# Pointcept/Pointcept

Measured on AMD Instinct MI355X. Metric: scenes/sec (fwd+bwd+optimizer) PTv3 ScanNet-semseg @ ~100k pts, higher is better.
Workload: dtype bf16; 1 GPU; PT-v3m1 base (46.2M params) + seg head + CE + Lovasz, fwd+bwd+AdamW, 8 scenes x 102400 voxels per GPU, patch 1024, 4 orders; global_batch=8, parallelism=dp1, params=46167572, amp=bf16 autocast, points_per_gpu=819200, loss=CrossEntropy(ignore_index=-1) + LovaszSoftmax

## Files before the change

pointcept_amd/csrc/lovasz.hip:

```cpp
#include "ptc_common.h"
#include "voxel_keys.h"
#include "loss_rows.h"

#define LV_THREADS 256
#define LV_MAX_C PTC_LOVASZ_DENSE_MAX_C
#define LV_ONE 0x3f800000u
#define LV_STEP_BLOCKS 4096

__device__ __forceinline__ int64_t lv_key(float e, bool fg) { return (int64_t)(((uint64_t)(LV_ONE - __float_as_uint(e)) << 1) | (fg ? 1u : 0u)); }
__device__ __forceinline__ float lv_key_error(int64_t key) { return __uint_as_float(LV_ONE - (uint32_t)((uint64_t)key >> 1)); }

template <typename T>
__global__ void __launch_bounds__(LV_THREADS)
lovasz_keys_kernel(const T* __restrict__ logits, int64_t row_stride, const int64_t* __restrict__ target, int64_t n, int c,
                   int64_t ignore_index, int64_t* __restrict__ keys, int32_t* __restrict__ class_count) {
  __shared__ int32_t cnt[LV_MAX_C];
  if (threadIdx.x < LV_MAX_C) cnt[threadIdx.x] = 0;
  __syncthreads();
  const int64_t i = (int64_t)blockIdx.x * LV_THREADS + threadIdx.x;
  if (i < n) {
    const T* row = logits + i * row_stride;
    const int64_t t = target[i];
    const bool valid = t != ignore_index && t >= 0 && t < c;
    float m = -INFINITY;
// ... 109 lines not shown
  __shared__ double red[LV_THREADS];
  double acc = 0.0;
  for (int64_t i = threadIdx.x; i < n_partial; i += LV_THREADS) acc += partial[i];
  red[threadIdx.x] = acc;
  __syncthreads();
  for (int s = LV_THREADS / 2; s >= 1; s >>= 1) {
    if ((int)threadIdx.x < s) red[threadIdx.x] += red[threadIdx.x + s];
    __syncthreads();
  }
  if (threadIdx.x == 0) {
    int np = 0;
    for (int j = 0; j < c; ++j) np += class_count[j] > 0 ? 1 : 0;
    loss[0] = np > 0 ? (float)(red[0] / (double)np) : 0.f;
  }
}

template <typename T>
__global__ void __launch_bounds__(LV_THREADS)
lovasz_dlogits_kernel(const T* __restrict__ logits, int64_t row_stride, const int64_t* __restrict__ target,
                      const float* __restrict__ gprob, int64_t n, int c, int64_t ignore_index, float* __restrict__ dlogits) {
  const int64_t i = (int64_t)blockIdx.x * LV_THREADS + threadIdx.x;
  if (i >= n) return;
  const T* row = logits + i * row_stride;
  float* drow = dlogits + i * (int64_t)c;
  const int64_t t = target[i];
  const bool valid = t != ignore_index && t >= 0 && t < c;
  if (!valid) {
    for (int j = 0; j < c; ++j) drow[j] = 0.f;
    return;
  }
  float m = -INFINITY;
  for (int j = 0; j < c; ++j) m = fmaxf(m, ptc_to_float(row[j]));
  float ssum = 0.f;
  for (int j = 0; j < c; ++j) ssum += __expf(ptc_to_float(row[j]) - m);
  const float inv = 1.f / ssum;
  float dot = 0.f;
  for (int j = 0; j < c; ++j) dot += gprob[(int64_t)j * n + i] * (__expf(ptc_to_float(row[j]) - m) * inv);
  for (int j = 0; j < c; ++j) {
    const float p = __expf(ptc_to_float(row[j]) - m) * inv;
    drow[j] = p * (gprob[(int64_t)j * n + i] - dot);
  }
}

template <typename T, int VB>
__global__ void __launch_bounds__(LV_THREADS)
lovasz_dlogits_rows_kernel(const T* __restrict__ logits, int64_t row_stride, const int64_t* __restrict__ target,
                           const float* __restrict__ gprob, int64_t n, int c, int64_t ignore_index, float* __restrict__ dlogits, int a16) {
  extern __shared__ __attribute__((aligned(16))) unsigned char smem[];
  const int64_t row0 = (int64_t)blockIdx.x * LV_THREADS, i = row0 + threadIdx.x;
  if (i < n) {
    float* drow = reinterpret_cast<float*>(smem) + (int)threadIdx.x * c;
    const int64_t t = target[i];
    const bool valid = t != ignore_index && t >= 0 && t < c;
    if (!valid) {
#pragma unroll
      for (int j = 0; j < LR_CP; ++j) if (j < c) drow[j] = 0.f;
    } else {
      float v[LR_CP], gp[LR_CP];
      lr_load_row<T, VB>(logits + i * row_stride, c, v);
#pragma unroll
      for (int j = 0; j < LR_CP; ++j) gp[j] = j < c ? gprob[(int64_t)j * n + i] : 0.f;
      float m = -INFINITY;
#pragma unroll
      for (int j = 0; j < LR_CP; ++j) if (j < c) m = fmaxf(m, v[j]);
      float ssum = 0.f;
#pragma unroll
      for (int j = 0; j < LR_CP; ++j) if (j < c) { v[j] = __expf(v[j] - m); ssum += v[j]; }
      const float inv = 1.f / ssum;
      float dot = 0.f;
#pragma unroll
      for (int j = 0; j < LR_CP; ++j) if (j < c) dot += gp[j] * (v[j] * inv);
#pragma unroll
      for (int j = 0; j < LR_CP; ++j) {
        if (j < c) {
          const float p = v[j] * inv;
          drow[j] = p * (gp[j] - dot);
        }
      }
    }
  }
  __syncthreads();
  const int64_t rows = (n - row0) < LV_THREADS ? (n - row0) : LV_THREADS;
  lr_copy_out<float>(smem, dlogits + row0 * c, (int)rows * c, a16 != 0);
}

struct LvLayout {
  size_t keys, order, fg, scan, gprob, partial, count, sort_ws, scan_ws, total;
  int64_t n_partial;
};
static LvLayout lv_layout(int64_t n, int c) {
  LvLayout L;
  const size_t nc = (size_t)(n > 0 ? n : 1) * (size_t)c;
  int64_t g = ptc_cdiv(n > 0 ? n : 1, LV_THREADS);
  if (g > LV_STEP_BLOCKS / c) g = LV_STEP_BLOCKS / c;
  L.n_partial = (g > 0 ? g : 1) * c;
  size_t o = 0;
  L.keys = o; o += ptc_align_up(nc * 8, 256);
  L.order = o; o += ptc_align_up(nc * 8, 256);
  L.fg = o; o += ptc_align_up(nc * 4, 256);
  L.scan = o; o += ptc_align_up(nc * 8, 256);
  L.gprob = o; o += ptc_align_up(nc * 4, 256);
  L.partial = o; o += ptc_align_up((size_t)L.n_partial * 8, 256);
  L.count = o; o += 256;
  L.sort_ws = o; o += ptc_align_up(ptc_sort_keys_workspace_bytes(n, c), 256);
  L.scan_ws = o; o += ptc_align_up(ptc_exclusive_scan_workspace_bytes((int64_t)nc), 256);
  L.total = o;
  return L;
}

extern "C" size_t ptc_lovasz_softmax_workspace_bytes(int64_t n, int c) {
  if (n < 0 || c < 1 || c > LV_MAX_C) return 0;
  return lv_layout(n, c).total;
}

extern "C" int ptc_lovasz_softmax(const void* logits, int64_t row_stride, const int64_t* target, int64_t n, int c, int dtype,
                                  int64_t ignore_index, float* loss, float* dlogits, void* workspace,
                                  size_t workspace_bytes, ptc_stream_t stream) {
  PTC_REQUIRE(n >= 0 && c >= 1 && row_stride >= c, PTC_EINVAL, "ptc_lovasz_softmax: bad sizes");
  PTC_REQUIRE(c <= LV_MAX_C, PTC_EUNSUPPORTED, "ptc_lovasz_softmax: c=%d > %d classes", c, LV_MAX_C);
  PTC_REQUIRE(n < (1ll << 31), PTC_EUNSUPPORTED, "ptc_lovasz_softmax: n >= 2^31");
  PTC_REQUIRE(loss != nullptr, PTC_EINVAL, "ptc_lovasz_softmax: null loss");
  hipStream_t s = (hipStream_t)stream;
  if (n == 0) {
    PTC_HIP(hipMemsetAsync(loss, 0, sizeof(float), s));
    return PTC_OK;
  }
  PTC_REQUIRE(logits && target && dlogits && workspace, PTC_EINVAL, "ptc_lovasz_softmax: null buffer");
  const LvLayout L = lv_layout(n, c);
  PTC_REQUIRE(workspace_bytes >= L.total, PTC_EWORKSPACE, "ptc_lovasz_softmax: workspace %zu < %zu", workspace_bytes, L.total);
  char* ws = (char*)workspace;
  int64_t* keys = (int64_t*)(ws + L.keys);
  int64_t* order = (int64_t*)(ws + L.order);
  int32_t* fg = (int32_t*)(ws + L.fg);
  int64_t* scan = (int64_t*)(ws + L.scan);
  float* gprob = (float*)(ws + L.gprob);
  double* partial = (double*)(ws + L.partial);
  int32_t* count = (int32_t*)(ws + L.count);
  const int64_t nc = n * (int64_t)c;
  const unsigned grid_n = (unsigned)ptc_cdiv(n, LV_THREADS), grid_nc = (unsigned)ptc_cdiv(nc, LV_THREADS);

  const bool rows = c <= LR_CP;
  const int vb = lr_vec_bytes(logits, row_stride, c, ptc_dtype_size(dtype));
  PTC_HIP(hipMemsetAsync(count, 0, 256, s));
  if (rows) {
    PTC_DISPATCH_DTYPE(dtype, T, LR_DISPATCH_VB(vb, VB, hipLaunchKernelGGL((lovasz_keys_rows_kernel<T, VB>), dim3(grid_n), dim3(LV_THREADS), 0, s,
                                                                         (const T*)logits, row_stride, target, n, c, ignore_index, keys, count)))
  } else {
    PTC_DISPATCH_DTYPE(dtype, T, hipLaunchKernelGGL(lovasz_keys_kernel<T>, dim3(grid_n), dim3(LV_THREADS), 0, s, (const T*)logits,
                                                     row_stride, target, n, c, ignore_index, keys, count))
  }
  PTC_CHECK_LAUNCH("lovasz_keys_kernel");
  int rc = ptc_sort_keys_ex(keys, n, c, 1, 31, order, nullptr, keys, ws + L.sort_ws, L.scan_ws - L.sort_ws, stream);
  if (rc != PTC_OK) return rc;
  hipLaunchKernelGGL(lovasz_fg_kernel, dim3(grid_nc), dim3(LV_THREADS), 0, s, keys, nc, fg);
  PTC_CHECK_LAUNCH("lovasz_fg_kernel");
  rc = ptc_exclusive_scan_i32(fg, nc, scan, ws + L.scan_ws, L.total - L.scan_ws, stream);
  if (rc != PTC_OK) return rc;
  hipLaunchKernelGGL(lovasz_step_kernel, dim3((unsigned)(L.n_partial / c), (unsigned)c), dim3(LV_THREADS), 0, s, keys, order, scan, count, n, c, gprob,
                     partial);
  PTC_CHECK_LAUNCH("lovasz_step_kernel");
  hipLaunchKernelGGL(lovasz_finish_kernel, dim3(1), dim3(LV_THREADS), 0, s, partial, L.n_partial, count, c, loss);
  PTC_CHECK_LAUNCH("lovasz_finish_kernel");
  if (rows) {
    const int a16 = ((uintptr_t)dlogits & 15) == 0;
    const size_t lds = (size_t)LV_THREADS * c * sizeof(float);
    PTC_DISPATCH_DTYPE(dtype, T, LR_DISPATCH_VB(vb, VB, hipLaunchKernelGGL((lovasz_dlogits_rows_kernel<T, VB>), dim3(grid_n), dim3(LV_THREADS), lds, s,
                                                                         (const T*)logits, row_stride, target, gprob, n, c, ignore_index, dlogits,
                                                                         a16)))
  } else {
    PTC_DISPATCH_DTYPE(dtype, T, hipLaunchKernelGGL(lovasz_dlogits_kernel<T>, dim3(grid_n), dim3(LV_THREADS), 0, s, (const T*)logits,
                                                     row_stride, target, gprob, n, c, ignore_index, dlogits))
  }
  PTC_CHECK_LAUNCH("lovasz_dlogits_kernel");
  return PTC_OK;
}

#define LW_MAX_C PTC_LOVASZ_MAX_C
#define LW_RV 16
#define LW_TILE_BYTES (32 * 1024)

__global__ void __launch_bounds__(LV_THREADS)
lovasz_count_kernel(const int64_t* __restrict__ target, int64_t n, int c, int64_t ignore_index, int32_t* __restrict__ class_count) {
  __shared__ int32_t cnt[LW_MAX_C];
  for (int j = threadIdx.x; j < c; j += LV_THREADS) cnt[j] = 0;
  __syncthreads();
  for (int64_t i = (int64_t)blockIdx.x * LV_THREADS + threadIdx.x; i < n; i += (int64_t)gridDim.x * LV_THREADS) {
    const int64_t t = target[i];
    if (t != ignore_index && t >= 0 && t < c) atomicAdd(&cnt[(int)t], 1);
  }
  __syncthreads();
  for (int j = threadIdx.x; j < c; j += LV_THREADS)
    if (cnt[j] != 0) atomicAdd(&class_count[j], cnt[j]);
}

__global__ void __launch_bounds__(LV_THREADS)
lovasz_rank_kernel(const int32_t* __restrict__ class_count, int c, int32_t* __restrict__ row_of, int32_t* __restrict__ class_of,
                   int32_t* __restrict__ n_present) {
  __shared__ int32_t wsum[LV_THREADS / 64];
  constexpr int PER = LW_MAX_C / LV_THREADS;
  const int lane = ptc_lane(), wave = threadIdx.x >> 6, j0 = (int)threadIdx.x * PER;
  bool f[PER];
  int32_t mine = 0;
#pragma unroll
  for (int q = 0; q < PER; ++q) {
    f[q] = j0 + q < c && class_count[j0 + q] > 0;
    mine += f[q] ? 1 : 0;
  }
  int32_t incl = mine;
#pragma unroll
  for (int o = 1; o < 64; o <<= 1) {
// ... 319 lines not shown
```

pointcept_amd/csrc/ptc_common.h:

```cpp
#pragma once
#include <hip/hip_runtime.h>
#include <stdint.h>
#include <stdio.h>
#include <stdarg.h>
#include "../../include/ptcore.h"

#define PTC_WAVE 64

void ptc_set_error(const char* fmt, ...);

#define PTC_REQUIRE(cond, code, ...)      \
  do {                                    \
    if (!(cond)) {                        \
      ptc_set_error(__VA_ARGS__);         \
      return (code);                      \
    }                                     \
  } while (0)

#define PTC_CHECK_LAUNCH(name)                                                        \
  do {                                                                                \
    hipError_t e__ = hipGetLastError();                                               \
    if (e__ != hipSuccess) {                                                          \
      ptc_set_error("%s: launch failed: %s", (name), hipGetErrorString(e__));         \
      return PTC_EHIP;                                                                \
// ... 54 lines not shown
#define PTC_DISPATCH_DTYPE(dtype, T, ...)                 \
  switch (dtype) {                                        \
    case PTC_F32: { using T = float; __VA_ARGS__; } break; \
    case PTC_F16: { using T = f16_t; __VA_ARGS__; } break; \
    case PTC_BF16: { using T = bf16_t; __VA_ARGS__; } break; \
    default: ptc_set_error("bad dtype %d", (int)(dtype)); return PTC_EINVAL; \
  }

static inline size_t ptc_dtype_size(int dtype) { return dtype == PTC_F32 ? 4 : 2; }

#define PTC_SWZ64(s) (((((s) >> 1) & 1) << 2) | (((s) >> 2) & 3))

__device__ __forceinline__ int ptc_lane() { return threadIdx.x & 63; }

__device__ __forceinline__ uint32_t ptc_float_enc(float f) {
  const uint32_t b = __float_as_uint(f);
  return (b & 0x80000000u) ? ~b : (b | 0x80000000u);
}
__device__ __forceinline__ float ptc_float_dec(uint32_t k) { return __uint_as_float((k & 0x80000000u) ? (k & 0x7fffffffu) : ~k); }

__device__ __forceinline__ float ptc_dist2(float ax, float ay, float az, float bx, float by, float bz) {
#pragma clang fp contract(off)
  const float dx = ax - bx, dy = ay - by, dz = az - bz;
  const float xx = dx * dx, yy = dy * dy, zz = dz * dz;
  return (xx + yy) + zz;
}

template <int I> struct ptc_int { static constexpr int value = I; };
template <int N, int I = 0, typename F> __device__ __forceinline__ void ptc_static_for(F&& f) {
  if constexpr (I < N) {
    f(ptc_int<I>{});
    ptc_static_for<N, I + 1>(f);
  }
}

__host__ __device__ __forceinline__ void ptc_rope_pair(float u, float v, float cs, float sn, float& ru, float& rv) {
  ru = fmaf(u, cs, -(v * sn));
  rv = fmaf(v, cs, u * sn);
}

#ifndef PTC_FAST_GELU
#define PTC_FAST_GELU 1
#endif
__device__ __forceinline__ float ptc_gelu_cdf(float z) {
#if PTC_FAST_GELU
  const float t = fminf(fabsf(z) * 0.70710678118654752f, 3.95f);
  float r = -4.535858889e-05f;
  r = fmaf(r, t, 4.455075312e-04f);
  r = fmaf(r, t, -1.489441160e-03f);
  r = fmaf(r, t, -7.746305554e-04f);
  r = fmaf(r, t, 2.825368195e-02f);
  r = fmaf(r, t, -1.484816155e-01f);
  r = fmaf(r, t, -9.184163932e-01f);
  r = fmaf(r, t, -1.627908593e+00f);
  const float h = __builtin_amdgcn_exp2f(fmaf(r, t, -1.0f));
  return z < 0.f ? h : 1.0f - h;
#else
  return 0.5f * (1.f + erff(z * 0.70710678118654752f));
#endif
}
__device__ __forceinline__ float ptc_gelu(float z) {
#if PTC_FAST_GELU
  return z * ptc_gelu_cdf(z);
#else
  return 0.5f * z * (1.f + erff(z * 0.70710678118654752f));
#endif
}
__device__ __forceinline__ float ptc_gelu_grad(float z) {
#if PTC_FAST_GELU
  return fmaf(z * 0.3989422804014327f, __builtin_amdgcn_exp2f(z * z * -0.72134752044448170f), ptc_gelu_cdf(z));
#else
  return 0.5f * (1.f + erff(z * 0.70710678118654752f)) + z * 0.3989422804014327f * __expf(-0.5f * z * z);
#endif
}

#ifdef __HIPCC__
#define PTC_WAVES_PER_EU(lo, hi) __attribute__((amdgpu_waves_per_eu(lo, hi)))
#else
#define PTC_WAVES_PER_EU(lo, hi)
#endif

int ptc_sort_keys_ex(const int64_t* keys, int64_t n, int k, int begin_bit, int end_bit, int64_t* order, int64_t* inverse,
                     int64_t* sorted_keys, void* workspace, size_t workspace_bytes, ptc_stream_t stream);
struct PtcCellGrid;
int ptc_cell_grid_params(const float* xyz, int64_t n, double radius, uint32_t* mm, PtcCellGrid* grid, ptc_stream_t stream);
int ptc_cell_grid_sort(const float* xyz, const int64_t* keys, int64_t n, int end_bit, int64_t* order, int64_t* sorted_keys, float4* sxyz,
                       void* scratch, size_t scratch_bytes, ptc_stream_t stream);
```

pointcept_amd/csrc/scan_sort.hip:

```cpp
#include "ptc_common.h"

__device__ __forceinline__ int64_t wave_inclusive_scan_i64(int64_t v) {
  const int lane = ptc_lane();
#pragma unroll
  for (int d = 1; d < 64; d <<= 1) {
    int lo = __shfl_up((int)(uint32_t)(v & 0xffffffffll), d, 64);
    int hi = __shfl_up((int)(uint32_t)((uint64_t)v >> 32), d, 64);
    int64_t o = (int64_t)(((uint64_t)(uint32_t)hi << 32) | (uint32_t)lo);
    if (lane >= d) v += o;
  }
  return v;
}

#define SCAN_THREADS 256
#define SCAN_ITEMS 8
#define SCAN_TILE (SCAN_THREADS * SCAN_ITEMS)

__device__ __forceinline__ int64_t block_exclusive_scan_i64(int64_t v, int64_t* total, int64_t* smem ) {
  const int lane = ptc_lane(), wave = threadIdx.x >> 6;
  int64_t inc = wave_inclusive_scan_i64(v);
  if (lane == 63) smem[wave] = inc;
  __syncthreads();
  if (threadIdx.x == 0) {
    int64_t run = 0;
    for (int w = 0; w < SCAN_THREADS / 64; ++w) { int64_t t = smem[w]; smem[w] = run; run += t; }
    smem[4] = run;
  }
  __syncthreads();
  int64_t excl = inc - v + smem[wave];
  *total = smem[4];
  __syncthreads();
  return excl;
}

__global__ void __launch_bounds__(SCAN_THREADS)
scan_tile_sums_kernel(const int32_t* __restrict__ in, int64_t n, int64_t* __restrict__ tile_sums) {
  __shared__ int64_t smem[5];
  const int64_t base = (int64_t)blockIdx.x * SCAN_TILE + (int64_t)threadIdx.x * SCAN_ITEMS;
  int64_t s = 0;
#pragma unroll
  for (int j = 0; j < SCAN_ITEMS; ++j) { int64_t i = base + j; if (i < n) s += in[i]; }
  int64_t total;
  block_exclusive_scan_i64(s, &total, smem);
  if (threadIdx.x == 0) tile_sums[blockIdx.x] = total;
}

__global__ void __launch_bounds__(SCAN_THREADS)
scan_tile_sums_scan_kernel(int64_t* __restrict__ tile_sums, int64_t n_tiles) {
  __shared__ int64_t smem[5];
  int64_t carry = 0;
  for (int64_t c = 0; c < n_tiles; c += SCAN_THREADS) {
    int64_t i = c + threadIdx.x;
    int64_t v = (i < n_tiles) ? tile_sums[i] : 0;
    int64_t total;
    int64_t ex = block_exclusive_scan_i64(v, &total, smem);
    if (i < n_tiles) tile_sums[i] = carry + ex;
    carry += total;
  }
}

__global__ void __launch_bounds__(SCAN_THREADS)
scan_apply_kernel(const int32_t* __restrict__ in, int64_t n, const int64_t* __restrict__ tile_offsets,
                  int64_t* __restrict__ out) {
  __shared__ int64_t smem[5];
  const int64_t base = (int64_t)blockIdx.x * SCAN_TILE + (int64_t)threadIdx.x * SCAN_ITEMS;
  int32_t v[SCAN_ITEMS];
  int64_t s = 0;
#pragma unroll
  for (int j = 0; j < SCAN_ITEMS; ++j) { int64_t i = base + j; v[j] = (i < n) ? in[i] : 0; s += v[j]; }
  int64_t total;
  int64_t ex = block_exclusive_scan_i64(s, &total, smem) + tile_offsets[blockIdx.x];
#pragma unroll
  for (int j = 0; j < SCAN_ITEMS; ++j) { int64_t i = base + j; if (i < n) out[i] = ex; ex += v[j]; }
}

#define SCAN1_THREADS 1024
#define SCAN1_ITEMS 16
#define SCAN1_MAX (SCAN1_THREADS * SCAN1_ITEMS)
__global__ void __launch_bounds__(SCAN1_THREADS)
scan_single_kernel(const int32_t* __restrict__ in, int64_t n, int64_t* __restrict__ out) {
  __shared__ int64_t wsum[SCAN1_THREADS / 64], wex[SCAN1_THREADS / 64 + 1];
  const int lane = ptc_lane(), wave = threadIdx.x >> 6;
  int64_t carry = 0;
  for (int64_t sweep = 0; sweep < n; sweep += (int64_t)SCAN1_THREADS * SCAN1_ITEMS) {
    const int64_t base = sweep + (int64_t)threadIdx.x * SCAN1_ITEMS;
    int32_t v[SCAN1_ITEMS];
    int64_t s = 0;
#pragma unroll
    for (int j = 0; j < SCAN1_ITEMS; ++j) { const int64_t i = base + j; v[j] = (i < n) ? in[i] : 0; s += v[j]; }
    const int64_t inc = wave_inclusive_scan_i64(s);
    if (lane == 63) wsum[wave] = inc;
    __syncthreads();
    if (wave == 0) {
      const int64_t w = lane < SCAN1_THREADS / 64 ? wsum[lane] : 0;
      const int64_t winc = wave_inclusive_scan_i64(w);
      if (lane < SCAN1_THREADS / 64) wex[lane] = winc - w;
      if (lane == SCAN1_THREADS / 64 - 1) wex[SCAN1_THREADS / 64] = winc;
    }
    __syncthreads();
    int64_t ex = carry + wex[wave] + inc - s;
#pragma unroll
    for (int j = 0; j < SCAN1_ITEMS; ++j) { const int64_t i = base + j; if (i < n) out[i] = ex; ex += v[j]; }
    carry += wex[SCAN1_THREADS / 64];
    __syncthreads();
  }
}

static int64_t scan_num_tiles(int64_t n) { return ptc_cdiv(n > 0 ? n : 1, SCAN_TILE); }

extern "C" size_t ptc_exclusive_scan_workspace_bytes(int64_t n) {
  return ptc_align_up((size_t)scan_num_tiles(n) * sizeof(int64_t), 256);
}

static int exclusive_scan_i32(const int32_t* in, int64_t n, int64_t* out, void* ws, hipStream_t s) {
  if (n <= 0) return PTC_OK;
  if (n <= SCAN1_MAX) {
    hipLaunchKernelGGL(scan_single_kernel, dim3(1), dim3(SCAN1_THREADS), 0, s, in, n, out);
    PTC_CHECK_LAUNCH("scan_single_kernel");
    return PTC_OK;
  }
  int64_t tiles = scan_num_tiles(n);
  int64_t* tile_sums = (int64_t*)ws;
  hipLaunchKernelGGL(scan_tile_sums_kernel, dim3((unsigned)tiles), dim3(SCAN_THREADS), 0, s, in, n, tile_sums);
  PTC_CHECK_LAUNCH("scan_tile_sums_kernel");
  hipLaunchKernelGGL(scan_tile_sums_scan_kernel, dim3(1), dim3(SCAN_THREADS), 0, s, tile_sums, tiles);
  PTC_CHECK_LAUNCH("scan_tile_sums_scan_kernel");
  hipLaunchKernelGGL(scan_apply_kernel, dim3((unsigned)tiles), dim3(SCAN_THREADS), 0, s, in, n, tile_sums, out);
  PTC_CHECK_LAUNCH("scan_apply_kernel");
  return PTC_OK;
}

extern "C" int ptc_exclusive_scan_i32(const int32_t* in, int64_t n, int64_t* out, void* workspace,
                                      size_t workspace_bytes, ptc_stream_t stream) {
  PTC_REQUIRE(n >= 0, PTC_EINVAL, "ptc_exclusive_scan_i32: n < 0");
  if (n == 0) return PTC_OK;
  PTC_REQUIRE(in && out && workspace, PTC_EINVAL, "ptc_exclusive_scan_i32: null buffer");
  PTC_REQUIRE(workspace_bytes >= ptc_exclusive_scan_workspace_bytes(n), PTC_EWORKSPACE,
              "ptc_exclusive_scan_i32: workspace %zu < %zu", workspace_bytes, ptc_exclusive_scan_workspace_bytes(n));
  return exclusive_scan_i32(in, n, out, workspace, (hipStream_t)stream);
}

#define RS_THREADS 256
#define RS_WAVES (RS_THREADS / 64)
#define RS_ITERS 16
#define RS_TILE (RS_THREADS * RS_ITERS)
#define RS_RADIX 256
#ifndef RS_PACK
#define RS_PACK 1
#endif

__device__ __forceinline__ uint32_t rs_digit(uint64_t key, int shift, uint32_t mask) {
  return (uint32_t)(key >> shift) & mask;
}

__global__ void __launch_bounds__(RS_THREADS)
rs_histogram_kernel(const uint64_t* __restrict__ keys, int64_t n, int shift, uint32_t mask,
                    int n_blocks, int32_t* __restrict__ hist) {
  __shared__ int32_t lh[RS_RADIX];
  const int row = blockIdx.y, blk = blockIdx.x;
  lh[threadIdx.x] = 0;
  __syncthreads();
  const uint64_t* k = keys + (int64_t)row * n;
  const int64_t base = (int64_t)blk * RS_TILE;
#pragma unroll 4
  for (int it = 0; it < RS_ITERS; ++it) {
    int64_t i = base + (int64_t)it * RS_THREADS + threadIdx.x;
    if (i < n) atomicAdd(&lh[rs_digit(k[i], shift, mask)], 1);
  }
  __syncthreads();
  hist[((int64_t)row * RS_RADIX + threadIdx.x) * n_blocks + blk] = lh[threadIdx.x];
}

template <bool FIRST, bool PACK>
__global__ void __launch_bounds__(RS_THREADS)
rs_scatter_kernel(const uint64_t* __restrict__ keys_in, const uint32_t* __restrict__ idx_in, int64_t n,
                  int shift, uint32_t mask, int n_blocks, const int64_t* __restrict__ offsets,
                  uint64_t* __restrict__ keys_out, uint32_t* __restrict__ idx_out, int idx_bits, uint64_t key_mask) {
  __shared__ int32_t wave_hist[RS_WAVES][RS_RADIX];
  __shared__ int64_t glob[RS_RADIX];
  __shared__ uint64_t skeys[RS_TILE];
  __shared__ uint32_t svals[PACK ? 1 : RS_TILE];
  const int row = blockIdx.y, blk = blockIdx.x;
  const int lane = ptc_lane(), wave = threadIdx.x >> 6;
  for (int i = threadIdx.x; i < RS_WAVES * RS_RADIX; i += RS_THREADS) (&wave_hist[0][0])[i] = 0;
  glob[threadIdx.x] = offsets[((int64_t)row * RS_RADIX + threadIdx.x) * n_blocks + blk] - (int64_t)row * n;
  __syncthreads();

  const uint64_t* k = keys_in + (int64_t)row * n;
  const uint32_t* ix = (FIRST || PACK) ? nullptr : idx_in + (int64_t)row * n;
  const int dshift = shift + ((PACK && FIRST) ? idx_bits : 0);
  const int64_t base = (int64_t)blk * RS_TILE + (int64_t)wave * (RS_ITERS * 64);
  const uint64_t lt_mask = (lane == 0) ? 0ull : (~0ull >> (64 - lane));

  uint64_t key[RS_ITERS];
  uint32_t val[RS_ITERS];
  int32_t rank[RS_ITERS];
#pragma unroll
  for (int it = 0; it < RS_ITERS; ++it) {
    const int64_t i = base + (int64_t)it * 64 + lane;
    const bool valid = i < n;
    key[it] = valid ? k[i] : ~0ull;
    if (PACK && FIRST && valid) key[it] = ((key[it] & key_mask) << idx_bits) | (uint64_t)i;
    val[it] = (valid && !PACK) ? (FIRST ? (uint32_t)i : ix[i]) : 0u;
    const uint32_t d = rs_digit(key[it], dshift, mask);
    uint64_t peers = __ballot(valid);
#pragma unroll
    for (int b = 0; b < 8; ++b) {
      const bool bit = (d >> b) & 1u;
      const uint64_t bal = __ballot(bit);
      peers &= bit ? bal : ~bal;
    }
    int32_t before = 0;
    if (valid) {
      before = wave_hist[wave][d];
      rank[it] = before + __popcll(peers & lt_mask);
    } else {
      rank[it] = 0;
    }
    __builtin_amdgcn_wave_barrier();
    if (valid && (peers & lt_mask) == 0ull) wave_hist[wave][d] = before + __popcll(peers);
    __builtin_amdgcn_wave_barrier();
  }
  __syncthreads();
  int32_t run = 0;
#pragma unroll
  for (int w = 0; w < RS_WAVES; ++w) { int32_t c = wave_hist[w][threadIdx.x]; wave_hist[w][threadIdx.x] = run; run += c; }
  __shared__ int32_t lstart[RS_RADIX];
  __shared__ int32_t wsum[RS_WAVES];
  {
    int32_t incl = run;
#pragma unroll
    for (int o = 1; o < 64; o <<= 1) {
      const int32_t v = __shfl_up(incl, o, 64);
      if (lane >= o) incl += v;
    }
    if (lane == 63) wsum[wave] = incl;
    __syncthreads();
    int32_t base_w = 0;
#pragma unroll
    for (int w = 0; w < RS_WAVES; ++w) base_w += (w < wave) ? wsum[w] : 0;
    lstart[threadIdx.x] = base_w + incl - run;
  }
  __syncthreads();
#pragma unroll
  for (int it = 0; it < RS_ITERS; ++it) {
    const int64_t i = base + (int64_t)it * 64 + lane;
    if (i < n) {
      const uint32_t d = rs_digit(key[it], dshift, mask);
      const int lp = lstart[d] + wave_hist[wave][d] + rank[it];
      skeys[lp] = key[it];
      if (!PACK) svals[lp] = val[it];
    }
  }
  __syncthreads();
  uint64_t* ko = keys_out + (int64_t)row * n;
  uint32_t* io = PACK ? nullptr : idx_out + (int64_t)row * n;
  const int64_t tile0 = (int64_t)blk * RS_TILE;
  const int cnt = (int)((n - tile0) < RS_TILE ? (n - tile0) : RS_TILE);
  for (int j = threadIdx.x; j < cnt; j += RS_THREADS) {
    const uint64_t kk = skeys[j];
// ... 1 lines not shown
    const int64_t dst = glob[d] + (j - lstart[d]);
    ko[dst] = kk;
    if (!PACK) io[dst] = svals[j];
  }
}

__global__ void __launch_bounds__(256)
rs_finalize_kernel(const uint32_t* __restrict__ idx, const uint64_t* __restrict__ packed, uint64_t idx_mask, int idx_bits, int64_t n, int k,
                   int64_t* __restrict__ order, int64_t* __restrict__ inverse, const uint64_t* plain,
                   int64_t* sorted_keys) {
  const int64_t total = n * k;
  const int64_t stride = (int64_t)gridDim.x * blockDim.x;
  for (int64_t t = (int64_t)blockIdx.x * blockDim.x + threadIdx.x; t < total; t += stride) {
    const int64_t row = t / n, i = t - row * n;
    const uint64_t word = packed ? packed[t] : 0ull;
    const int64_t src = packed ? (int64_t)(word & idx_mask) : (idx ? (int64_t)idx[t] : i);
    order[t] = src;
    if (inverse) inverse[row * n + src] = i;
    if (sorted_keys) sorted_keys[t] = (int64_t)(packed ? (word >> idx_bits) : plain[t]);
  }
}

static int rs_num_blocks(int64_t n) { return (int)ptc_cdiv(n > 0 ? n : 1, RS_TILE); }

struct RsLayout {
  size_t keysA, keysB, idxA, idxB, hist, offs, scan, total;
};
static RsLayout rs_layout(int64_t n, int k) {
  RsLayout L;
  const size_t nk = (size_t)(n > 0 ? n : 1) * (size_t)k;
  const size_t nh = (size_t)k * RS_RADIX * (size_t)rs_num_blocks(n);
  size_t o = 0;
  L.keysA = o; o += ptc_align_up(nk * 8, 256);
  L.keysB = o; o += ptc_align_up(nk * 8, 256);
  L.idxA = o; o += ptc_align_up(nk * 4, 256);
  L.idxB = o; o += ptc_align_up(nk * 4, 256);
  L.hist = o; o += ptc_align_up(nh * 4, 256);
  L.offs = o; o += ptc_align_up(nh * 8, 256);
  L.scan = o; o += ptc_exclusive_scan_workspace_bytes((int64_t)nh);
  L.total = o;
  return L;
}

extern "C" size_t ptc_sort_keys_workspace_bytes(int64_t n, int k) { return rs_layout(n, k).total; }

extern "C" int ptc_sort_keys(const int64_t* keys, int64_t n, int k, int begin_bit, int end_bit,
                             int64_t* order, int64_t* inverse, void* workspace, size_t workspace_bytes,
                             ptc_stream_t stream) {
  return ptc_sort_keys_ex(keys, n, k, begin_bit, end_bit, order, inverse, nullptr, workspace, workspace_bytes, stream);
}

int ptc_sort_keys_ex(const int64_t* keys, int64_t n, int k, int begin_bit, int end_bit, int64_t* order, int64_t* inverse,
                     int64_t* sorted_keys, void* workspace, size_t workspace_bytes, ptc_stream_t stream) {
  PTC_REQUIRE(n >= 0 && k >= 1, PTC_EINVAL, "ptc_sort_keys: bad n=%lld k=%d", (long long)n, k);
  PTC_REQUIRE(begin_bit >= 0 && end_bit <= 64 && begin_bit <= end_bit, PTC_EINVAL,
              "ptc_sort_keys: bad bit range [%d,%d)", begin_bit, end_bit);
  PTC_REQUIRE(n < (1ll << 32), PTC_EUNSUPPORTED, "ptc_sort_keys: n >= 2^32");
  if (n == 0) return PTC_OK;
  PTC_REQUIRE(keys && order && workspace, PTC_EINVAL, "ptc_sort_keys: null buffer");
  const RsLayout L = rs_layout(n, k);
  PTC_REQUIRE(workspace_bytes >= L.total, PTC_EWORKSPACE, "ptc_sort_keys: workspace %zu < %zu", workspace_bytes, L.total);
  hipStream_t s = (hipStream_t)stream;
  char* ws = (char*)workspace;
  uint64_t* kbuf[2] = {(uint64_t*)(ws + L.keysA), (uint64_t*)(ws + L.keysB)};
  uint32_t* ibuf[2] = {(uint32_t*)(ws + L.idxA), (uint32_t*)(ws + L.idxB)};
  int32_t* hist = (int32_t*)(ws + L.hist);
  int64_t* offs = (int64_t*)(ws + L.offs);
  void* scan_ws = ws + L.scan;
  const int nb = rs_num_blocks(n);
  const int64_t nh = (int64_t)k * RS_RADIX * nb;

  const uint64_t* cur_k = (const uint64_t*)keys;
  const uint32_t* cur_i = nullptr;
  int out = 0;
  bool first = true;
  int idx_bits = 1;
  while (((int64_t)1 << idx_bits) < n) ++idx_bits;
  const bool pack = RS_PACK && (end_bit - begin_bit) > 0 && end_bit + idx_bits <= 64;
  const uint64_t key_mask = end_bit >= 64 ? ~0ull : (((uint64_t)1 << end_bit) - 1);
  for (int shift = begin_bit; shift < end_bit; shift += 8) {
    const int bits = (end_bit - shift) < 8 ? (end_bit - shift) : 8;
    const uint32_t mask = (1u << bits) - 1u;
    const int hshift = shift + ((pack && !first) ? idx_bits : 0);
    hipLaunchKernelGGL(rs_histogram_kernel, dim3(nb, k), dim3(RS_THREADS), 0, s, cur_k, n, hshift, mask, nb, hist);
    PTC_CHECK_LAUNCH("rs_histogram_kernel");
    int rc = exclusive_scan_i32(hist, nh, offs, scan_ws, s);
    if (rc != PTC_OK) return rc;
#define RS_SCATTER(F, P)                                                                                                                          \
    hipLaunchKernelGGL((rs_scatter_kernel<F, P>), dim3(nb, k), dim3(RS_THREADS), 0, s, cur_k, cur_i, n, (P && !F) ? shift + idx_bits : shift, mask, nb, \
                       offs, kbuf[out], ibuf[out], idx_bits, key_mask)
    if (pack) { if (first) RS_SCATTER(true, true); else RS_SCATTER(false, true); }
    else { if (first) RS_SCATTER(true, false); else RS_SCATTER(false, false); }
#undef RS_SCATTER
    PTC_CHECK_LAUNCH("rs_scatter_kernel");
    cur_k = kbuf[out];
    cur_i = ibuf[out];
    out ^= 1;
    first = false;
  }
  {
    const int64_t total = n * k;
    int64_t grid = ptc_cdiv(total, 256);
    if (grid > 4096) grid = 4096;
    const bool packed_out = pack && !first;
    hipLaunchKernelGGL(rs_finalize_kernel, dim3((unsigned)grid), dim3(256), 0, s, packed_out ? nullptr : cur_i, packed_out ? cur_k : nullptr,
                       (((uint64_t)1 << idx_bits) - 1), idx_bits, n, k, order, inverse, cur_k, sorted_keys);
    PTC_CHECK_LAUNCH("rs_finalize_kernel");
  }
  return PTC_OK;
}
```

Before: 229.7 scenes/s.

## Compact Lovasz sort to live entries and use single flat device-sized radix sort

Adds a flat Lovasz-softmax path. For each class it computes a cutoff, the minimum error among that class's foreground points. Only entries at or above that cutoff (plus foreground entries) are compacted into packed 64-bit words (class | error | fg | index), which are then sorted with a radix sort whose length comes from a device-side count. This replaces the full n*c per-class key sort, since entries below the cutoff contribute no Lovasz gradient, and it cuts the sort from many per-class rows to one packed pass over the live subset. The cost is extra passes over the logits (cut, live count, compaction), added small scans and launches, and correctness that depends on the cutoff argument and on the bit packing fitting in 64 bits.

```diff
diff --git a/pointcept_amd/csrc/lovasz.hip b/pointcept_amd/csrc/lovasz.hip
--- a/pointcept_amd/csrc/lovasz.hip
+++ b/pointcept_amd/csrc/lovasz.hip
@@ -215,6 +215,337 @@
   __syncthreads();
   const int64_t rows = (n - row0) < LV_THREADS ? (n - row0) : LV_THREADS;
   lr_copy_out<float>(smem, dlogits + row0 * c, (int)rows * c, a16 != 0);
+}
+
+struct LvState {
+  int32_t count[LV_MAX_C];
+  int32_t live[LV_MAX_C];
+  uint32_t cut[LV_MAX_C];
+  int64_t seg_start[LV_MAX_C];
+  int32_t fg_start[LV_MAX_C];
+  int64_t m;
+  int32_t n_present;
+};
+#define LF_ITEMS 8
+#define LF_TILE (LV_THREADS * LF_ITEMS)
+
+__device__ __forceinline__ void lv_row_errors(float (&v)[LR_CP], int c, int64_t t, bool valid) {
+  float m = -INFINITY;
+#pragma unroll
+  for (int j = 0; j < LR_CP; ++j) if (j < c) m = fmaxf(m, v[j]);
+  float ssum = 0.f;
+#pragma unroll
+  for (int j = 0; j < LR_CP; ++j) if (j < c) { v[j] = __expf(v[j] - m); ssum += v[j]; }
+  const float inv = 1.f / ssum;
+#pragma unroll
+  for (int j = 0; j < LR_CP; ++j) {
+    if (j < c) {
+      const float p = v[j] * inv;
+      const float e = valid ? (j == t ? 1.f - p : p) : 0.f;
+      v[j] = fminf(fmaxf(e, 0.f), 1.f);
+    }
+  }
+}
+
+__device__ __forceinline__ uint32_t lv_live_mask(const float (&e)[LR_CP], int c, int64_t t, bool valid, const uint32_t* cut) {
+  uint32_t mask = 0;
+#pragma unroll
+  for (int j = 0; j < LR_CP; ++j)
+    if (j < c && ((valid && j == t) || __float_as_uint(e[j]) >= cut[j])) mask |= 1u << j;
+  return mask;
+}
+
+template <typename T, int VB>
+__global__ void __launch_bounds__(LV_THREADS)
+lovasz_cut_kernel(const T* __restrict__ logits, int64_t row_stride, const int64_t* __restrict__ target, int64_t n, int c,
+                  int64_t ignore_index, LvState* __restrict__ st) {
+  __shared__ int32_t cnt[LR_CP];
+  __shared__ uint32_t cut[LR_CP];
+  if (threadIdx.x < LR_CP) { cnt[threadIdx.x] = 0; cut[threadIdx.x] = 0xffffffffu; }
+  __syncthreads();
+  const int64_t i = (int64_t)blockIdx.x * LV_THREADS + threadIdx.x;
+  if (i < n) {
+    const int64_t t = target[i];
+    if (t != ignore_index && t >= 0 && t < c) {
+      float v[LR_CP];
+      lr_load_row<T, VB>(logits + i * row_stride, c, v);
+      lv_row_errors(v, c, t, true);
+      atomicAdd(&cnt[(int)t], 1);
+      atomicMin(&cut[(int)t], __float_as_uint(lr_pick(v, (int)t)));
+    }
+  }
+  __syncthreads();
+  if (threadIdx.x < c && cnt[threadIdx.x] != 0) {
+    atomicAdd(&st->count[threadIdx.x], cnt[threadIdx.x]);
+    atomicMin(&st->cut[threadIdx.x], cut[threadIdx.x]);
+  }
+}
+
+template <typename T, int VB>
+__global__ void __launch_bounds__(LV_THREADS)
+lovasz_live_count_kernel(const T* __restrict__ logits, int64_t row_stride, const int64_t* __restrict__ target, int64_t n, int c,
+                         int64_t ignore_index, LvState* __restrict__ st, int32_t* __restrict__ block_live) {
+  __shared__ int32_t lc[LR_CP];
+  __shared__ uint32_t cut[LR_CP];
+  if (threadIdx.x < LR_CP) { lc[threadIdx.x] = 0; cut[threadIdx.x] = threadIdx.x < c ? st->cut[threadIdx.x] : 0xffffffffu; }
+  __syncthreads();
+  const int64_t i = (int64_t)blockIdx.x * LV_THREADS + threadIdx.x;
+  uint32_t mask = 0;
+  if (i < n) {
+    float v[LR_CP];
+    lr_load_row<T, VB>(logits + i * row_stride, c, v);
+    const int64_t t = target[i];
+    const bool valid = t != ignore_index && t >= 0 && t < c;
+    lv_row_errors(v, c, t, valid);
+    mask = lv_live_mask(v, c, t, valid, cut);
+  }
+  for (int j = 0; j < c; ++j) {
+    const uint64_t b = __ballot((mask >> j) & 1u);
+    if (ptc_lane() == 0 && b != 0ull) atomicAdd(&lc[j], __popcll(b));
+  }
+  __syncthreads();
+  if (threadIdx.x < c && lc[threadIdx.x] != 0) atomicAdd(&st->live[threadIdx.x], lc[threadIdx.x]);
+  if (threadIdx.x == 0) {
+    int32_t total = 0;
+    for (int j = 0; j < c; ++j) total += lc[j];
+    block_live[blockIdx.x] = total;
+  }
+}
+
+__global__ void lovasz_plan_kernel(LvState* __restrict__ st, int c) {
+  int64_t seg = 0;
+  int32_t fg = 0, np = 0;
+  for (int j = 0; j < c; ++j) {
+    st->seg_start[j] = seg;
+    st->fg_start[j] = fg;
+    seg += st->live[j];
+    fg += st->count[j];
+    np += st->count[j] > 0 ? 1 : 0;
+  }
+  st->m = seg;
+  st->n_present = np;
+}
+
+template <typename T, int VB>
+__global__ void __launch_bounds__(LV_THREADS)
+lovasz_compact_kernel(const T* __restrict__ logits, int64_t row_stride, const int64_t* __restrict__ target, int64_t n, int c,
+                      int64_t ignore_index, const LvState* __restrict__ st, const int64_t* __restrict__ block_off, int pbits,
+                      int64_t cap, uint64_t* __restrict__ words) {
+  __shared__ uint32_t cut[LR_CP];
+  __shared__ int32_t wsum[LV_THREADS / 64];
+  if (threadIdx.x < LR_CP) cut[threadIdx.x] = threadIdx.x < c ? st->cut[threadIdx.x] : 0xffffffffu;
+  __syncthreads();
+  const int64_t i = (int64_t)blockIdx.x * LV_THREADS + threadIdx.x;
+  const int lane = ptc_lane(), wave = threadIdx.x >> 6;
+  float v[LR_CP];
+  uint32_t mask = 0;
+  int64_t t = -1;
+  bool valid = false;
+  if (i < n) {
+    lr_load_row<T, VB>(logits + i * row_stride, c, v);
+    t = target[i];
+    valid = t != ignore_index && t >= 0 && t < c;
+    lv_row_errors(v, c, t, valid);
+    mask = lv_live_mask(v, c, t, valid, cut);
+  }
+  const int32_t mine = __popc(mask);
+  int32_t incl = mine;
+#pragma unroll
+  for (int o = 1; o < 64; o <<= 1) {
+    const int32_t u = __shfl_up(incl, o, 64);
+    if (lane >= o) incl += u;
+  }
+  if (lane == 63) wsum[wave] = incl;
+  __syncthreads();
+  int32_t before = 0;
+#pragma unroll
+  for (int w = 0; w < LV_THREADS / 64; ++w) before += w < wave ? wsum[w] : 0;
+  int64_t o = block_off[blockIdx.x] + before + incl - mine;
+  if (o + mine > cap) return;
+#pragma unroll
+  for (int j = 0; j < LR_CP; ++j) {
+    if (j < c && ((mask >> j) & 1u)) {
+      const uint64_t key = ((uint64_t)j << 31) | ((uint64_t)(LV_ONE - __float_as_uint(v[j])) << 1) | ((valid && j == t) ? 1u : 0u);
+      words[o++] = (key << pbits) | (uint64_t)i;
+    }
+  }
+}
+
+__global__ void __launch_bounds__(LV_THREADS)
+lovasz_tile_fg_kernel(const uint64_t* __restrict__ sorted, const LvState* __restrict__ st, int pbits, int32_t* __restrict__ tile_fg) {
+  __shared__ int32_t red[LV_THREADS / 64];
+  const int64_t m = st->m, tile0 = (int64_t)blockIdx.x * LF_TILE;
+  if (tile0 >= m) {
+    if (threadIdx.x == 0) tile_fg[blockIdx.x] = 0;
+    return;
+  }
+  int32_t s = 0;
+#pragma unroll
+  for (int it = 0; it < LF_ITEMS; ++it) {
+    const int64_t i = tile0 + it * LV_THREADS + threadIdx.x;
+    if (i < m) s += (int32_t)((sorted[i] >> pbits) & 1ull);
+  }
+#pragma unroll
+  for (int o = 32; o >= 1; o >>= 1) s += __shfl_xor(s, o, 64);
+  if (ptc_lane() == 0) red[threadIdx.x >> 6] = s;
+  __syncthreads();
+  if (threadIdx.x == 0) tile_fg[blockIdx.x] = (red[0] + red[1]) + (red[2] + red[3]);
+}
+
+__global__ void __launch_bounds__(LV_THREADS)
+lovasz_step_flat_kernel(const uint64_t* __restrict__ sorted, const LvState* __restrict__ st, const int64_t* __restrict__ tile_off, int64_t n,
+                        int c, int pbits, float* __restrict__ gprob, double* __restrict__ partial) {
+  __shared__ double red[LV_THREADS / 64];
+  __shared__ int32_t wtot[LV_THREADS / 64];
+  __shared__ int64_t seg0[LR_CP];
+  __shared__ int32_t fg0[LR_CP], gts_s[LR_CP];
+  const int64_t m = st->m, tile0 = (int64_t)blockIdx.x * LF_TILE;
+  if (tile0 >= m) {
+    if (threadIdx.x == 0) partial[blockIdx.x] = 0.0;
+    return;
+  }
+  if ((int)threadIdx.x < c) {
+    seg0[threadIdx.x] = st->seg_start[threadIdx.x];
+    fg0[threadIdx.x] = st->fg_start[threadIdx.x];
+    gts_s[threadIdx.x] = st->count[threadIdx.x];
+  }
+  const double inv_present = 1.0 / (double)st->n_present;
+  const int lane = ptc_lane(), wave = threadIdx.x >> 6;
+  const uint64_t lt_mask = (lane == 0) ? 0ull : (~0ull >> (64 - lane));
+  const uint64_t pmask = ((uint64_t)1 << pbits) - 1;
+  const int64_t base = tile0 + (int64_t)wave * (LF_ITEMS * 64);
+  uint64_t w[LF_ITEMS];
+  int32_t before[LF_ITEMS];
+  int32_t run = 0;
+#pragma unroll
+  for (int it = 0; it < LF_ITEMS; ++it) {
+    const int64_t i = base + it * 64 + lane;
+    w[it] = i < m ? sorted[i] : 0ull;
+    const uint64_t bal = __ballot((int)((w[it] >> pbits) & 1ull));
+    before[it] = run + __popcll(bal & lt_mask);
+    run += __popcll(bal);
+  }
+  if (lane == 0) wtot[wave] = run;
+  __syncthreads();
+  int64_t cum0 = tile_off[blockIdx.x];
+#pragma unroll
+  for (int k = 0; k < LV_THREADS / 64; ++k) cum0 += k < wave ? wtot[k] : 0;
+  double contrib = 0.0;
+#pragma unroll
+  for (int it = 0; it < LF_ITEMS; ++it) {
+    const int64_t i = base + it * 64 + lane;
+    if (i < m) {
+      const int cls = (int)(w[it] >> (pbits + 31));
+      const int64_t src = (int64_t)(w[it] & pmask);
+      if (cls < c && src < n) {
+        const int64_t key = (int64_t)((w[it] >> pbits) & 0x7fffffffull);
+        contrib += lv_step_slot(key, (int32_t)src, (int32_t)(cum0 + before[it] - fg0[cls]), (int32_t)(i - seg0[cls]), gts_s[cls],
+                                inv_present, gprob + (int64_t)cls * n);
+      }
+    }
+  }
+#pragma unroll
+  for (int o = 32; o >= 1; o >>= 1) contrib += __shfl_xor(contrib, o, 64);
+  if (lane == 0) red[wave] = contrib;
+  __syncthreads();
+  if (threadIdx.x == 0) partial[blockIdx.x] = (red[0] + red[1]) + (red[2] + red[3]);
+}
+
+static int lv_bits(int64_t v) {
+  int b = 0;
+  while (((int64_t)1 << b) < v) ++b;
+  return b;
+}
+#ifndef LV_FLAT
+#define LV_FLAT 1
+#endif
+static bool lv_flat(int64_t n, int c) {
+  return LV_FLAT && c <= LR_CP && n >= 1 && n * (int64_t)c < (1ll << 32) && lv_bits(c) + 31 + (lv_bits(n) > 0 ? lv_bits(n) : 1) <= 64;
+}
+
+struct LfLayout {
+  size_t words_a, words_b, gprob, block_live, block_off, tile_fg, tile_off, partial, state, sort_ws, scan_ws, total;
+  int64_t n_blocks, n_tiles;
+};
+static LfLayout lf_layout(int64_t n, int c) {
+  LfLayout L;
+  const size_t nc = (size_t)n * (size_t)c;
+  L.n_blocks = ptc_cdiv(n, LV_THREADS);
+  L.n_tiles = ptc_cdiv((int64_t)nc, LF_TILE);
+  size_t o = 0;
+  L.words_a = o; o += ptc_align_up(nc * 8, 256);
+  L.words_b = o; o += ptc_align_up(nc * 8, 256);
+  L.gprob = o; o += ptc_align_up(nc * 4, 256);
+  L.block_live = o; o += ptc_align_up((size_t)L.n_blocks * 4, 256);
+  L.block_off = o; o += ptc_align_up((size_t)L.n_blocks * 8, 256);
+  L.tile_fg = o; o += ptc_align_up((size_t)L.n_tiles * 4, 256);
+  L.tile_off = o; o += ptc_align_up((size_t)L.n_tiles * 8, 256);
+  L.partial = o; o += ptc_align_up((size_t)L.n_tiles * 8, 256);
+  L.state = o; o += ptc_align_up(sizeof(LvState), 256);
+  L.sort_ws = o; o += ptc_align_up(ptc_sort_words_dev_workspace_bytes((int64_t)nc), 256);
+  const int64_t ns = L.n_blocks > L.n_tiles ? L.n_blocks : L.n_tiles;
+  L.scan_ws = o; o += ptc_align_up(ptc_exclusive_scan_workspace_bytes(ns), 256);
+  L.total = o;
+  return L;
+}
+
+static int lv_softmax_flat(const void* logits, int64_t row_stride, const int64_t* target, int64_t n, int c, int dtype, int64_t ignore_index,
+                           float* loss, float* dlogits, void* workspace, size_t workspace_bytes, ptc_stream_t stream) {
+  hipStream_t s = (hipStream_t)stream;
+  const LfLayout L = lf_layout(n, c);
+  PTC_REQUIRE(workspace_bytes >= L.total, PTC_EWORKSPACE, "ptc_lovasz_softmax: workspace %zu < %zu", workspace_bytes, L.total);
+  char* ws = (char*)workspace;
+  uint64_t* words_a = (uint64_t*)(ws + L.words_a);
+  uint64_t* words_b = (uint64_t*)(ws + L.words_b);
+  float* gprob = (float*)(ws + L.gprob);
+  int32_t* block_live = (int32_t*)(ws + L.block_live);
+  int64_t* block_off = (int64_t*)(ws + L.block_off);
+  int32_t* tile_fg = (int32_t*)(ws + L.tile_fg);
+  int64_t* tile_off = (int64_t*)(ws + L.tile_off);
+  double* partial = (double*)(ws + L.partial);
+  LvState* st = (LvState*)(ws + L.state);
+  const int64_t nc = n * (int64_t)c;
+  const unsigned grid_n = (unsigned)L.n_blocks, grid_t = (unsigned)L.n_tiles;
+  const int pbits = lv_bits(n) > 0 ? lv_bits(n) : 1, cbits = lv_bits(c);
+  const int vb = lr_vec_bytes(logits, row_stride, c, ptc_dtype_size(dtype));
+  const size_t scan_bytes = L.total - L.scan_ws;
+
+  PTC_HIP(hipMemsetAsync(st, 0, sizeof(LvState), s));
+  PTC_HIP(hipMemsetAsync(st->cut, 0xff, sizeof(st->cut), s));
+  PTC_HIP(hipMemsetAsync(gprob, 0, (size_t)nc * sizeof(float), s));
+  PTC_DISPATCH_DTYPE(dtype, T, LR_DISPATCH_VB(vb, VB, hipLaunchKernelGGL((lovasz_cut_kernel<T, VB>), dim3(grid_n), dim3(LV_THREADS), 0, s,
+                                                                       (const T*)logits, row_stride, target, n, c, ignore_index, st)))
+  PTC_CHECK_LAUNCH("lovasz_cut_kernel");
+  PTC_DISPATCH_DTYPE(dtype, T, LR_DISPATCH_VB(vb, VB, hipLaunchKernelGGL((lovasz_live_count_kernel<T, VB>), dim3(grid_n), dim3(LV_THREADS), 0, s,
+                                                                       (const T*)logits, row_stride, target, n, c, ignore_index, st,
+                                                                       block_live)))
+  PTC_CHECK_LAUNCH("lovasz_live_count_kernel");
+  int rc = ptc_exclusive_scan_i32(block_live, L.n_blocks, block_off, ws + L.scan_ws, scan_bytes, stream);
+  if (rc != PTC_OK) return rc;
+  hipLaunchKernelGGL(lovasz_plan_kernel, dim3(1), dim3(1), 0, s, st, c);
+  PTC_CHECK_LAUNCH("lovasz_plan_kernel");
+  PTC_DISPATCH_DTYPE(dtype, T, LR_DISPATCH_VB(vb, VB, hipLaunchKernelGGL((lovasz_compact_kernel<T, VB>), dim3(grid_n), dim3(LV_THREADS), 0, s,
+                                                                       (const T*)logits, row_stride, target, n, c, ignore_index, st, block_off,
+                                                                       pbits, nc, words_a)))
+  PTC_CHECK_LAUNCH("lovasz_compact_kernel");
+  uint64_t* sorted = nullptr;
+  rc = ptc_sort_words_dev(words_a, words_b, nc, &st->m, pbits + 1, pbits + 31 + cbits, &sorted, ws + L.sort_ws, L.scan_ws - L.sort_ws, stream);
+  if (rc != PTC_OK) return rc;
+  hipLaunchKernelGGL(lovasz_tile_fg_kernel, dim3(grid_t), dim3(LV_THREADS), 0, s, sorted, st, pbits, tile_fg);
+  PTC_CHECK_LAUNCH("lovasz_tile_fg_kernel");
+  rc = ptc_exclusive_scan_i32(tile_fg, L.n_tiles, tile_off, ws + L.scan_ws, scan_bytes, stream);
+  if (rc != PTC_OK) return rc;
+  hipLaunchKernelGGL(lovasz_step_flat_kernel, dim3(grid_t), dim3(LV_THREADS), 0, s, sorted, st, tile_off, n, c, pbits, gprob, partial);
+  PTC_CHECK_LAUNCH("lovasz_step_flat_kernel");
+  hipLaunchKernelGGL(lovasz_finish_kernel, dim3(1), dim3(LV_THREADS), 0, s, partial, L.n_tiles, st->count, c, loss);
+  PTC_CHECK_LAUNCH("lovasz_finish_kernel");
+  const int a16 = ((uintptr_t)dlogits & 15) == 0;
+  const size_t lds = (size_t)LV_THREADS * c * sizeof(float);
+  PTC_DISPATCH_DTYPE(dtype, T, LR_DISPATCH_VB(vb, VB, hipLaunchKernelGGL((lovasz_dlogits_rows_kernel<T, VB>), dim3(grid_n), dim3(LV_THREADS), lds, s,
+                                                                       (const T*)logits, row_stride, target, gprob, n, c, ignore_index, dlogits,
+                                                                       a16)))
+  PTC_CHECK_LAUNCH("lovasz_dlogits_kernel");
+  return PTC_OK;
 }
 
 struct LvLayout {
@@ -243,6 +574,7 @@
 
 extern "C" size_t ptc_lovasz_softmax_workspace_bytes(int64_t n, int c) {
   if (n < 0 || c < 1 || c > LV_MAX_C) return 0;
+  if (lv_flat(n, c)) return lf_layout(n, c).total;
   return lv_layout(n, c).total;
 }
 
@@ -259,6 +591,7 @@
     return PTC_OK;
   }
   PTC_REQUIRE(logits && target && dlogits && workspace, PTC_EINVAL, "ptc_lovasz_softmax: null buffer");
+  if (lv_flat(n, c)) return lv_softmax_flat(logits, row_stride, target, n, c, dtype, ignore_index, loss, dlogits, workspace, workspace_bytes, stream);
   const LvLayout L = lv_layout(n, c);
   PTC_REQUIRE(workspace_bytes >= L.total, PTC_EWORKSPACE, "ptc_lovasz_softmax: workspace %zu < %zu", workspace_bytes, L.total);
   char* ws = (char*)workspace;
diff --git a/pointcept_amd/csrc/ptc_common.h b/pointcept_amd/csrc/ptc_common.h
--- a/pointcept_amd/csrc/ptc_common.h
+++ b/pointcept_amd/csrc/ptc_common.h
@@ -160,6 +160,9 @@
 
 int ptc_sort_keys_ex(const int64_t* keys, int64_t n, int k, int begin_bit, int end_bit, int64_t* order, int64_t* inverse,
                      int64_t* sorted_keys, void* workspace, size_t workspace_bytes, ptc_stream_t stream);
+size_t ptc_sort_words_dev_workspace_bytes(int64_t cap);
+int ptc_sort_words_dev(uint64_t* a, uint64_t* b, int64_t cap, const int64_t* n_dev, int begin_bit, int end_bit, uint64_t** sorted,
+                       void* workspace, size_t workspace_bytes, ptc_stream_t stream);
 struct PtcCellGrid;
 int ptc_cell_grid_params(const float* xyz, int64_t n, double radius, uint32_t* mm, PtcCellGrid* grid, ptc_stream_t stream);
 int ptc_cell_grid_sort(const float* xyz, const int64_t* keys, int64_t n, int end_bit, int64_t* order, int64_t* sorted_keys, float4* sxyz,
diff --git a/pointcept_amd/csrc/scan_sort.hip b/pointcept_amd/csrc/scan_sort.hip
--- a/pointcept_amd/csrc/scan_sort.hip
+++ b/pointcept_amd/csrc/scan_sort.hip
@@ -33,9 +33,18 @@
   return excl;
 }
 
+__device__ __forceinline__ int64_t scan_dev_len(const int64_t* __restrict__ n_dev, int64_t bound) {
+  const int64_t v = n_dev[0];
+  return v < 0 ? 0 : (v < bound ? v : bound);
+}
+
 __global__ void __launch_bounds__(SCAN_THREADS)
-scan_tile_sums_kernel(const int32_t* __restrict__ in, int64_t n, int64_t* __restrict__ tile_sums) {
+scan_tile_sums_kernel(const int32_t* __restrict__ in, int64_t n, int64_t* __restrict__ tile_sums, const int64_t* __restrict__ n_dev) {
   __shared__ int64_t smem[5];
+  if (n_dev) {
+    n = scan_dev_len(n_dev, n);
+    if ((int64_t)blockIdx.x * SCAN_TILE >= n) return;
+  }
   const int64_t base = (int64_t)blockIdx.x * SCAN_TILE + (int64_t)threadIdx.x * SCAN_ITEMS;
   int64_t s = 0;
 #pragma unroll
@@ -46,8 +55,9 @@
 }
 
 __global__ void __launch_bounds__(SCAN_THREADS)
-scan_tile_sums_scan_kernel(int64_t* __restrict__ tile_sums, int64_t n_tiles) {
+scan_tile_sums_scan_kernel(int64_t* __restrict__ tile_sums, int64_t n_tiles, const int64_t* __restrict__ n_dev) {
   __shared__ int64_t smem[5];
+  if (n_dev) n_tiles = (scan_dev_len(n_dev, n_tiles * SCAN_TILE) + SCAN_TILE - 1) / SCAN_TILE;
   int64_t carry = 0;
   for (int64_t c = 0; c < n_tiles; c += SCAN_THREADS) {
     int64_t i = c + threadIdx.x;
@@ -61,8 +71,12 @@
 
 __global__ void __launch_bounds__(SCAN_THREADS)
 scan_apply_kernel(const int32_t* __restrict__ in, int64_t n, const int64_t* __restrict__ tile_offsets,
-                  int64_t* __restrict__ out) {
+                  int64_t* __restrict__ out, const int64_t* __restrict__ n_dev) {
   __shared__ int64_t smem[5];
+  if (n_dev) {
+    n = scan_dev_len(n_dev, n);
+    if ((int64_t)blockIdx.x * SCAN_TILE >= n) return;
+  }
   const int64_t base = (int64_t)blockIdx.x * SCAN_TILE + (int64_t)threadIdx.x * SCAN_ITEMS;
   int32_t v[SCAN_ITEMS];
   int64_t s = 0;
@@ -112,20 +126,20 @@
   return ptc_align_up((size_t)scan_num_tiles(n) * sizeof(int64_t), 256);
 }
 
-static int exclusive_scan_i32(const int32_t* in, int64_t n, int64_t* out, void* ws, hipStream_t s) {
+static int exclusive_scan_i32(const int32_t* in, int64_t n, int64_t* out, void* ws, hipStream_t s, const int64_t* n_dev = nullptr) {
   if (n <= 0) return PTC_OK;
-  if (n <= SCAN1_MAX) {
+  if (n <= SCAN1_MAX && !n_dev) {
     hipLaunchKernelGGL(scan_single_kernel, dim3(1), dim3(SCAN1_THREADS), 0, s, in, n, out);
     PTC_CHECK_LAUNCH("scan_single_kernel");
     return PTC_OK;
   }
   int64_t tiles = scan_num_tiles(n);
   int64_t* tile_sums = (int64_t*)ws;
-  hipLaunchKernelGGL(scan_tile_sums_kernel, dim3((unsigned)tiles), dim3(SCAN_THREADS), 0, s, in, n, tile_sums);
+  hipLaunchKernelGGL(scan_tile_sums_kernel, dim3((unsigned)tiles), dim3(SCAN_THREADS), 0, s, in, n, tile_sums, n_dev);
   PTC_CHECK_LAUNCH("scan_tile_sums_kernel");
-  hipLaunchKernelGGL(scan_tile_sums_scan_kernel, dim3(1), dim3(SCAN_THREADS), 0, s, tile_sums, tiles);
+  hipLaunchKernelGGL(scan_tile_sums_scan_kernel, dim3(1), dim3(SCAN_THREADS), 0, s, tile_sums, tiles, n_dev);
   PTC_CHECK_LAUNCH("scan_tile_sums_scan_kernel");
-  hipLaunchKernelGGL(scan_apply_kernel, dim3((unsigned)tiles), dim3(SCAN_THREADS), 0, s, in, n, tile_sums, out);
+  hipLaunchKernelGGL(scan_apply_kernel, dim3((unsigned)tiles), dim3(SCAN_THREADS), 0, s, in, n, tile_sums, out, n_dev);
   PTC_CHECK_LAUNCH("scan_apply_kernel");
   return PTC_OK;
 }
@@ -155,9 +169,14 @@
 
 __global__ void __launch_bounds__(RS_THREADS)
 rs_histogram_kernel(const uint64_t* __restrict__ keys, int64_t n, int shift, uint32_t mask,
-                    int n_blocks, int32_t* __restrict__ hist) {
+                    int n_blocks, int32_t* __restrict__ hist, const int64_t* __restrict__ n_dev) {
   __shared__ int32_t lh[RS_RADIX];
   const int row = blockIdx.y, blk = blockIdx.x;
+  if (n_dev) {
+    n = scan_dev_len(n_dev, n);
+    n_blocks = (int)((n + RS_TILE - 1) / RS_TILE);
+    if (blk >= n_blocks) return;
+  }
   lh[threadIdx.x] = 0;
   __syncthreads();
   const uint64_t* k = keys + (int64_t)row * n;
@@ -175,7 +194,13 @@
 __global__ void __launch_bounds__(RS_THREADS)
 rs_scatter_kernel(const uint64_t* __restrict__ keys_in, const uint32_t* __restrict__ idx_in, int64_t n,
                   int shift, uint32_t mask, int n_blocks, const int64_t* __restrict__ offsets,
-                  uint64_t* __restrict__ keys_out, uint32_t* __restrict__ idx_out, int idx_bits, uint64_t key_mask) {
+                  uint64_t* __restrict__ keys_out, uint32_t* __restrict__ idx_out, int idx_bits, uint64_t key_mask,
+                  const int64_t* __restrict__ n_dev) {
+  if (n_dev) {
+    n = scan_dev_len(n_dev, n);
+    n_blocks = (int)((n + RS_TILE - 1) / RS_TILE);
+    if ((int)blockIdx.x >= n_blocks) return;
+  }
   __shared__ int32_t wave_hist[RS_WAVES][RS_RADIX];
   __shared__ int64_t glob[RS_RADIX];
   __shared__ uint64_t skeys[RS_TILE];
@@ -343,13 +368,13 @@
     const int bits = (end_bit - shift) < 8 ? (end_bit - shift) : 8;
     const uint32_t mask = (1u << bits) - 1u;
     const int hshift = shift + ((pack && !first) ? idx_bits : 0);
-    hipLaunchKernelGGL(rs_histogram_kernel, dim3(nb, k), dim3(RS_THREADS), 0, s, cur_k, n, hshift, mask, nb, hist);
+    hipLaunchKernelGGL(rs_histogram_kernel, dim3(nb, k), dim3(RS_THREADS), 0, s, cur_k, n, hshift, mask, nb, hist, nullptr);
     PTC_CHECK_LAUNCH("rs_histogram_kernel");
     int rc = exclusive_scan_i32(hist, nh, offs, scan_ws, s);
     if (rc != PTC_OK) return rc;
 #define RS_SCATTER(F, P)                                                                                                                          \
     hipLaunchKernelGGL((rs_scatter_kernel<F, P>), dim3(nb, k), dim3(RS_THREADS), 0, s, cur_k, cur_i, n, (P && !F) ? shift + idx_bits : shift, mask, nb, \
-                       offs, kbuf[out], ibuf[out], idx_bits, key_mask)
+                       offs, kbuf[out], ibuf[out], idx_bits, key_mask, nullptr)
     if (pack) { if (first) RS_SCATTER(true, true); else RS_SCATTER(false, true); }
     else { if (first) RS_SCATTER(true, false); else RS_SCATTER(false, false); }
 #undef RS_SCATTER
@@ -370,3 +395,61 @@
   }
   return PTC_OK;
 }
+
+__global__ void rs_dev_sizes_kernel(const int64_t* __restrict__ n_dev, int64_t cap, int64_t* __restrict__ sizes) {
+  const int64_t n = scan_dev_len(n_dev, cap);
+  sizes[0] = n;
+  sizes[1] = (n + RS_TILE - 1) / RS_TILE * RS_RADIX;
+}
+
+struct RsDevLayout {
+  size_t hist, offs, scan, sizes, total;
+};
+static RsDevLayout rs_dev_layout(int64_t cap) {
+  RsDevLayout L;
+  const size_t nh = (size_t)RS_RADIX * (size_t)rs_num_blocks(cap);
+  size_t o = 0;
+  L.hist = o; o += ptc_align_up(nh * 4, 256);
+  L.offs = o; o += ptc_align_up(nh * 8, 256);
+  L.scan = o; o += ptc_exclusive_scan_workspace_bytes((int64_t)nh);
+  L.sizes = o; o += 256;
+  L.total = o;
+  return L;
+}
+
+size_t ptc_sort_words_dev_workspace_bytes(int64_t cap) { return rs_dev_layout(cap).total; }
+
+int ptc_sort_words_dev(uint64_t* a, uint64_t* b, int64_t cap, const int64_t* n_dev, int begin_bit, int end_bit, uint64_t** sorted,
+                       void* workspace, size_t workspace_bytes, ptc_stream_t stream) {
+  PTC_REQUIRE(cap >= 1 && cap < (1ll << 32), PTC_EINVAL, "ptc_sort_words_dev: bad cap=%lld", (long long)cap);
+  PTC_REQUIRE(begin_bit >= 0 && end_bit <= 64 && begin_bit <= end_bit, PTC_EINVAL, "ptc_sort_words_dev: bad bit range [%d,%d)", begin_bit,
+              end_bit);
+  PTC_REQUIRE(a && b && n_dev && sorted && workspace, PTC_EINVAL, "ptc_sort_words_dev: null buffer");
+  const RsDevLayout L = rs_dev_layout(cap);
+  PTC_REQUIRE(workspace_bytes >= L.total, PTC_EWORKSPACE, "ptc_sort_words_dev: workspace %zu < %zu", workspace_bytes, L.total);
+  hipStream_t s = (hipStream_t)stream;
+  char* ws = (char*)workspace;
+  int32_t* hist = (int32_t*)(ws + L.hist);
+  int64_t* offs = (int64_t*)(ws + L.offs);
+  int64_t* sizes = (int64_t*)(ws + L.sizes);
+  const int nb = rs_num_blocks(cap);
+  const int64_t nh = (int64_t)RS_RADIX * nb;
+  hipLaunchKernelGGL(rs_dev_sizes_kernel, dim3(1), dim3(1), 0, s, n_dev, cap, sizes);
+  PTC_CHECK_LAUNCH("rs_dev_sizes_kernel");
+  uint64_t* cur = a;
+  uint64_t* other = b;
+  for (int shift = begin_bit; shift < end_bit; shift += 8) {
+    const int bits = (end_bit - shift) < 8 ? (end_bit - shift) : 8;
+    const uint32_t mask = (1u << bits) - 1u;
+    hipLaunchKernelGGL(rs_histogram_kernel, dim3(nb, 1), dim3(RS_THREADS), 0, s, cur, cap, shift, mask, nb, hist, sizes);
+    PTC_CHECK_LAUNCH("rs_histogram_kernel");
+    int rc = exclusive_scan_i32(hist, nh, offs, ws + L.scan, s, sizes + 1);
+    if (rc != PTC_OK) return rc;
+    hipLaunchKernelGGL((rs_scatter_kernel<false, true>), dim3(nb, 1), dim3(RS_THREADS), 0, s, cur, nullptr, cap, shift, mask, nb, offs, other,
+                       nullptr, 0, ~0ull, sizes);
+    PTC_CHECK_LAUNCH("rs_scatter_kernel");
+    uint64_t* t = cur; cur = other; other = t;
+  }
+  *sorted = cur;
+  return PTC_OK;
+}
```

Measured after the change: 228.5 scenes/s. About the same (-0.5%).
